# Intelligent-Driving-Laboratory/GOPS

Hardware: AMD Instinct MI355X
Metric: env-model steps/sec (batch x H), FHADP compute_gradient + update (higher is better)
Workload: dtype f32; 1 GPU; target_veh3dof_fhadp_b4096_h30; env_id=pyth_veh3dofconti, algorithm=FHADP, batch_per_gpu=4096, horizon=30, activation=elu, parallelism=dp1

## Files before the change

### gops_amd/csrc/aux_kernels.hip

```cpp
#include <algorithm>
#include "common.h"
#include "env_models.h"
#include "launchers.h"

__device__ __forceinline__ void pack_element(const float* __restrict__ W, int N, int K, int Kp,
                                             float* __restrict__ wp, float* __restrict__ wpt, int e) {
    if (e >= N * Kp) return;
    const int i = e & 3, lane = (e >> 2) & 63, blk = e >> 8;
    {
        const int kch = Kp >> 4, nt = blk / kch, c = blk - nt * kch;
        const int n = 16 * nt + (lane & 15), k = 16 * c + 4 * (lane >> 4) + i;
        wp[e] = (k < K) ? W[(size_t)n * K + k] : 0.f;
    }
    {
        const int kch = N >> 4, nt = blk / kch, c = blk - nt * kch;
        const int kin = 16 * nt + (lane & 15), nout = 16 * c + 4 * (lane >> 4) + i;
        wpt[e] = (kin < K) ? W[(size_t)nout * K + kin] : 0.f;
    }
}

__device__ __forceinline__ void pack_element_h(const float* __restrict__ W, int N, int K, int Kp16, int Kp32, int layer,
                                               _Float16* __restrict__ wph, _Float16* __restrict__ wpth, int e) {
    const int i8 = e & 7, lane = (e >> 3) & 63, blk = e >> 9, r = lane & 15, kg = lane >> 4;
    if (e < N * Kp32) {
// ... 417 lines not shown
        const f32x4 zero4 = {0.f, 0.f, 0.f, 0.f};
        if constexpr (BF3) {
            bf16x8 b[R][3];
#pragma unroll
            for (int j = 0; j < R; ++j) {
                split_frag(xra[j][0], LAST_HALF_EMPTY ? zero4 : xra[j][1], b[j]);
                load_x(next_blk, j);
            }
#pragma unroll
            for (int i = 0; i < R; ++i) {
                const f32x4 d0 = dra[i][0], d1 = LAST_HALF_EMPTY ? zero4 : dra[i][1];
                bf16x8 a[3];
                split_frag(d0, d1, a);
                bsum[i] += ((d0[0] + d0[1]) + (d0[2] + d0[3])) + ((d1[0] + d1[1]) + (d1[2] + d1[3]));
                load_d(next_blk, i);
                constexpr int PA[6] = {2, 0, 1, 1, 0, 0}, PB[6] = {0, 2, 1, 0, 1, 0};
#pragma unroll
                for (int q = 0; q < 6; ++q)
#pragma unroll
                    for (int j = 0; j < R; ++j)
                        acc[i][j] = __builtin_amdgcn_mfma_f32_16x16x32_bf16(a[PA[q]], b[j][PB[q]], acc[i][j], 0, 0, 0);
            }
        } else {
            f32x4 xc[R][2];
#pragma unroll
            for (int j = 0; j < R; ++j) {
                xc[j][0] = xra[j][0]; xc[j][1] = LAST_HALF_EMPTY ? zero4 : xra[j][1];
                load_x(next_blk, j);
            }
#pragma unroll
            for (int i = 0; i < R; ++i) {
                const f32x4 d0 = dra[i][0], d1 = LAST_HALF_EMPTY ? zero4 : dra[i][1];
                bsum[i] += ((d0[0] + d0[1]) + (d0[2] + d0[3])) + ((d1[0] + d1[1]) + (d1[2] + d1[3]));
                load_d(next_blk, i);
#pragma unroll
                for (int u = 0; u < 8; ++u)
#pragma unroll
                    for (int j = 0; j < R; ++j)
                        acc[i][j] = __builtin_amdgcn_mfma_f32_16x16x4f32(u < 4 ? d0[u & 3] : d1[u & 3], xc[j][u >> 2][u & 3], acc[i][j], 0, 0, 0);
            }
        }
    };

#pragma unroll
    for (int j = 0; j < R; ++j) load_x(blk_of(0), j);
#pragma unroll
    for (int i = 0; i < R; ++i) load_d(blk_of(0), i);
    const int nfull = odd_tail ? nblk - 1 : nblk;
    for (int c = 0; c < nfull; ++c) block.template operator()<false>(blk_of(c + 1));
    if (odd_tail) block.template operator()<true>(blk_of(nblk));
    float* pbase = part + (size_t)split * N * Kp;
#pragma unroll
    for (int i = 0; i < R; ++i)
#pragma unroll
        for (int j = 0; j < R; ++j) {
            const int k = kb + 16 * j + f;
#pragma unroll
            for (int r = 0; r < 4; ++r) {
                const int n = nb + 16 * i + 4 * g + r;
                if (n < N && k < Kp) pbase[(size_t)n * Kp + k] = acc[i][j][r];
            }
        }
    if (want_bias) {
#pragma unroll
        for (int i = 0; i < R; ++i) {
            float t = bsum[i];
            t += __shfl_xor(t, 16);
            t += __shfl_xor(t, 32);
            if (g == 0 && nb + 16 * i + f < N) part_b[(size_t)split * N + nb + 16 * i + f] = t;
        }
    }
}

#define DW_H2_SA 1.0f
#define DW_H2_LO 1.0f
__device__ __forceinline__ void split2h(const f32x4& lo4, const f32x4& hi4, float s, f16x8& ph, f16x8& pl) {
    const float s2 = s * DW_H2_LO;
    u32x4 uh, ul;
#pragma unroll
    for (int e = 0; e < 4; ++e) {
        const float x0 = e < 2 ? lo4[2 * e] : hi4[2 * e - 4], x1 = e < 2 ? lo4[2 * e + 1] : hi4[2 * e - 3];
        const f16x2 h = __builtin_bit_cast(f16x2, __builtin_amdgcn_cvt_pkrtz(x0 * s, x1 * s));
        const float r0 = fmaf((float)h[0], -DW_H2_LO, x0 * s2), r1 = fmaf((float)h[1], -DW_H2_LO, x1 * s2);
        uh[e] = __builtin_bit_cast(unsigned, h);
        ul[e] = __builtin_bit_cast(unsigned, __builtin_amdgcn_cvt_pkrtz(r0, r1));
    }
    ph = __builtin_bit_cast(f16x8, uh);
    pl = __builtin_bit_cast(f16x8, ul);
}

__device__ __forceinline__ void split2h_mix(const f32x4& lo4, const f32x4& hi4, float s, f16x8& ph, f16x8& pl) {
    u32x4 uh, ul;
#pragma unroll
    for (int e = 0; e < 4; ++e) {
        const float x0 = e < 2 ? lo4[2 * e] : hi4[2 * e - 4], x1 = e < 2 ? lo4[2 * e + 1] : hi4[2 * e - 3];
        unsigned h, l;
        asm("v_fma_mixlo_f16 %0, %1, %2, 0" : "=v"(h) : "v"(s), "v"(x0));
        asm("v_fma_mixhi_f16 %0, %1, %2, 0" : "+v"(h) : "v"(s), "v"(x1));
        asm("v_fma_mixlo_f16 %0, %1, %2, -%3 op_sel_hi:[0,0,1]" : "=v"(l) : "v"(s), "v"(x0), "v"(h));
        asm("v_fma_mixhi_f16 %0, %1, %2, -%3 op_sel:[0,0,1] op_sel_hi:[0,0,1]" : "+v"(l) : "v"(s), "v"(x1), "v"(h));
        uh[e] = h;
        ul[e] = l;
    }
    ph = __builtin_bit_cast(f16x8, uh);
    pl = __builtin_bit_cast(f16x8, ul);
}
__device__ __forceinline__ void absmax2(float& m, float a, float b) { asm("v_max3_f32 %0, |%1|, |%2|, %0" : "+v"(m) : "v"(a), "v"(b)); }

__device__ __forceinline__ float dw_delta_yardstick(const float* dscale) {
    const float dy = gptr(dscale)[1], gv = gptr(dscale)[0];
    return dy > 0.f ? dy : gv;
}

#define DWR_STAGES 2
#define DWR_STAGE_FLOATS (4 * 2048)

template <bool H2>
__global__ __launch_bounds__(NTHREADS, 2) void dw_gemm_ring_kernel(const float* __restrict__ D, int N,
                                                                    const float* __restrict__ X, int Kp,
                                                                    long long Q, int splits, int chunks_per_split,
                                                                    float* __restrict__ part,
                                                                    float* __restrict__ part_b, const float* __restrict__ dscale, int redo_guard) {
    extern __shared__ __attribute__((aligned(16))) float ring[];
    constexpr int T = 128, R = 4;
    const int tid = threadIdx.x, lane = tid & 63, wave = tid >> 6;
    const int tiles_k = (Kp + T - 1) / T, tiles = tiles_k * (N / T);
    const int xcd = blockIdx.x & 7, local = blockIdx.x >> 3;
    const int tile = local % tiles, split = (local / tiles) * 8 + xcd;
    if (split >= splits) return;
    const int tile_n = tile / tiles_k, tile_k = tile - tile_n * tiles_k;
    const int wn = wave >> 1, wk = wave & 1;
    const int f = lane & 15, g = lane >> 4;
    const bool want_bias = part_b != nullptr && tile_k == 0 && wk == 0;
    const long long nblk_all = (Q + 1) >> 1;
    const int nblk = (int)((nblk_all - split + splits - 1) / splits);
    const bool odd_tail = (Q & 1) && ((nblk_all - 1) % splits == split);

    const float* csrc = (wave < 2) ? D + (size_t)tile_n * T * 16 : X + (size_t)tile_k * T * 16;
    const size_t ctile = (size_t)((wave < 2) ? N : Kp) * 16;
    const int kvalid = (wave < 2) ? T : min(T, Kp - tile_k * T);
    auto copy_block = [&](int c, int stage) {
        const long long bq = min(((long long)split + (long long)min(c, nblk - 1) * splits) * 2 + (wave & 1), Q - 1);
        const float* src = csrc + (size_t)bq * ctile + 4 * lane;
        const float* dst = ring + stage * DWR_STAGE_FLOATS + wave * 2048;
#pragma unroll
        for (int u = 0; u < 8; ++u) {
            const int feat = u * 16 + (lane >> 2);
            async_copy16_to_lds<true>(feat < kvalid ? src + u * 256 : src + u * 256 - (size_t)(feat - (feat % kvalid)) * 16, dst + u * 256);
        }
    };

    f32x4 acc[R][R] = {};
    float bsum[R] = {0.f, 0.f, 0.f, 0.f};
    float sd = 1.f;
    if constexpr (H2) sd = f16_grad_scale(dw_delta_yardstick(dscale)) * 16.f;
    auto block = [&]<bool LAST_HALF_EMPTY, bool M2>(int stage) {
        const float* st = ring + stage * DWR_STAGE_FLOATS;
        const float* da = st + (wn * 64 + f) * 16 + 4 * g;
        const float* xa = st + 4096 + (wk * 64 + f) * 16 + 4 * g;
        const f32x4 zero4 = {0.f, 0.f, 0.f, 0.f};
        if constexpr (M2) {
            f16x8 bh[R], bl[R];
#pragma unroll
            for (int j = 0; j < R; ++j) {
                bh[j] = *reinterpret_cast<const f16x8*>(xa + 256 * j);
                bl[j] = *reinterpret_cast<const f16x8*>(xa + 256 * j + 2048);
            }
#pragma unroll
            for (int i = 0; i < R; ++i) {
                const f16x8 ah = *reinterpret_cast<const f16x8*>(da + 256 * i), al = *reinterpret_cast<const f16x8*>(da + 256 * i + 2048);
#pragma unroll
                for (int j = 0; j < R; ++j) acc[i][j] = __builtin_amdgcn_mfma_f32_16x16x32_f16(al, bh[j], acc[i][j], 0, 0, 0);
#pragma unroll
                for (int j = 0; j < R; ++j) acc[i][j] = __builtin_amdgcn_mfma_f32_16x16x32_f16(ah, bl[j], acc[i][j], 0, 0, 0);
#pragma unroll
                for (int j = 0; j < R; ++j) acc[i][j] = __builtin_amdgcn_mfma_f32_16x16x32_f16(ah, bh[j], acc[i][j], 0, 0, 0);
            }
            return;
        }
        bf16x8 b[R][3];
#pragma unroll
        for (int j = 0; j < R; ++j) {
            const f32x4 x0 = *reinterpret_cast<const f32x4*>(xa + 256 * j);
            const f32x4 x1 = LAST_HALF_EMPTY ? zero4 : *reinterpret_cast<const f32x4*>(xa + 256 * j + 2048);
            split_frag(x0, x1, b[j]);
        }
#pragma unroll
        for (int i = 0; i < R; ++i) {
            const f32x4 d0 = *reinterpret_cast<const f32x4*>(da + 256 * i);
            const f32x4 d1 = LAST_HALF_EMPTY ? zero4 : *reinterpret_cast<const f32x4*>(da + 256 * i + 2048);
            bf16x8 a[3];
            split_frag(d0, d1, a);
            bsum[i] += ((d0[0] + d0[1]) + (d0[2] + d0[3])) + ((d1[0] + d1[1]) + (d1[2] + d1[3]));
            constexpr int PA[6] = {2, 0, 1, 1, 0, 0}, PB[6] = {0, 2, 1, 0, 1, 0};
#pragma unroll
            for (int q = 0; q < 6; ++q)
#pragma unroll
                for (int j = 0; j < R; ++j)
                    acc[i][j] = __builtin_amdgcn_mfma_f32_16x16x32_bf16(a[PA[q]], b[j][PB[q]], acc[i][j], 0, 0, 0);
        }
    };

    float vmax = 0.f;
    float csum[2] = {0.f, 0.f};
    auto convert_stage = [&]<bool LAST_HALF_EMPTY>(int stage) {
        float* st = ring + stage * DWR_STAGE_FLOATS;
#pragma unroll
        for (int k = 0; k < 4; ++k) {
            const int id = tid + NTHREADS * k, op = id >> 9, fe = (id >> 2) & 127, gg = id & 3;
            float* at = st + op * 4096 + fe * 16 + 4 * gg;
            const f32x4 v0 = *reinterpret_cast<const f32x4*>(at);
            const f32x4 zero4 = {0.f, 0.f, 0.f, 0.f};
            const f32x4 v1 = LAST_HALF_EMPTY ? zero4 : *reinterpret_cast<const f32x4*>(at + 2048);
            if (k < 2) csum[k] += ((v0[0] + v0[1]) + (v0[2] + v0[3])) + ((v1[0] + v1[1]) + (v1[2] + v1[3]));
            const float sc = k < 2 ? sd : DW_H2_SA;
            const float m0 = fmaxf(fmaxf(fabsf(v0[0]), fabsf(v0[1])), fmaxf(fabsf(v0[2]), fabsf(v0[3])));
            const float m1 = fmaxf(fmaxf(fabsf(v1[0]), fabsf(v1[1])), fmaxf(fabsf(v1[2]), fabsf(v1[3])));
            vmax = fmaxf(vmax, fmaxf(m0, m1) * sc);
            f16x8 ph, pl;
            split2h(v0, v1, sc, ph, pl);
            *reinterpret_cast<f16x8*>(at) = ph;
            *reinterpret_cast<f16x8*>(at + 2048) = pl;
        }
    };
    const int nfull = odd_tail ? nblk - 1 : nblk;
    auto run = [&]<bool M2>() {
#pragma unroll
        for (int d = 0; d < DWR_STAGES - 1; ++d) copy_block(d, d);
        for (int c = 0; c < nblk; ++c) {
            asm volatile("s_waitcnt vmcnt(%0)" ::"n"(8 * (DWR_STAGES - 2)) : "memory");
            __syncthreads();
            copy_block(c + DWR_STAGES - 1, (c + DWR_STAGES - 1) % DWR_STAGES);
            if constexpr (M2) {
                if (c < nfull) convert_stage.template operator()<false>(c % DWR_STAGES);
                else convert_stage.template operator()<true>(c % DWR_STAGES);
                __syncthreads();
            }
            if (c < nfull) block.template operator()<false, M2>(c % DWR_STAGES);
            else block.template operator()<true, M2>(c % DWR_STAGES);
        }
        asm volatile("s_waitcnt vmcnt(0)" ::: "memory");
    };
    bool redone = false;
    if constexpr (H2) {
        if (tid == 0) ring[DWR_STAGES * DWR_STAGE_FLOATS] = 0.f;
        run.template operator()<true>();
        unsigned* sat = reinterpret_cast<unsigned*>(ring + DWR_STAGES * DWR_STAGE_FLOATS);
        if (!(vmax < 65504.f)) *sat = 1u;
        __syncthreads();
        if (*sat != 0u && redo_guard) {
            redone = true;
#pragma unroll
            for (int i = 0; i < R; ++i)
#pragma unroll
                for (int j = 0; j < R; ++j) acc[i][j] = f32x4{0.f, 0.f, 0.f, 0.f};
            run.template operator()<false>();
        }
    } else {
        run.template operator()<false>();
    }

    const int nb = tile_n * T + wn * 64, kb = tile_k * T + wk * 64;
    float* pbase = part + (size_t)split * N * Kp;
    const float unscale = (H2 && !redone) ? 1.f / (sd * DW_H2_SA) : 1.f;
#pragma unroll
    for (int i = 0; i < R; ++i)
#pragma unroll
        for (int j = 0; j < R; ++j) {
            const int k = kb + 16 * j + f;
            if (k >= Kp) continue;
#pragma unroll
            for (int r = 0; r < 4; ++r) {
                float v = acc[i][j][r];
                if constexpr (H2) v *= unscale;
                pbase[(size_t)(nb + 16 * i + 4 * g + r) * Kp + k] = v;
            }
        }
    if constexpr (H2) {
        if (part_b != nullptr && tile_k == 0) {
#pragma unroll
            for (int k = 0; k < 2; ++k) {
                float t = csum[k];
                t += __shfl_xor(t, 1);
                t += __shfl_xor(t, 2);
                if ((tid & 3) == 0) part_b[(size_t)split * N + tile_n * T + 64 * k + (tid >> 2)] = t;
            }
        }
    } else
    if (want_bias) {
#pragma unroll
        for (int i = 0; i < R; ++i) {
            float t = bsum[i];
            t += __shfl_xor(t, 16);
            t += __shfl_xor(t, 32);
            if (g == 0) part_b[(size_t)split * N + nb + 16 * i + f] = t;
        }
    }
}

struct DwSpec {
    static constexpr int NW = 8, NT = 512, TN = 256, T = 128;
    static constexpr int DT = TN * 16;
    static constexpr int STAGES = 3;
    static constexpr int STAGE_FLOATS = 2 * DT + 4096;
    static constexpr int PIECES = STAGE_FLOATS / 256 / NW;
    static constexpr size_t lds_bytes() { return (size_t)STAGES * STAGE_FLOATS * sizeof(float) + 16; }
};

struct DwSpecGeo {
    const float* dbase;
    const float* xbase;
    float* pbase;
    long long Q;
    int N, Kp, split, splits, nblk, nfull, xgroups, tile_n, tile_k;
};
__device__ __forceinline__ void dw_spec_copy(const DwSpecGeo& G, float* ring, int c, int stage, int wave, int lane) {
    constexpr int T = DwSpec::T, TN = DwSpec::TN, PC = DwSpec::PIECES;
    const long long b0 = ((long long)G.split + (long long)c * G.splits) * 2;
    float* dst = ring + stage * DwSpec::STAGE_FLOATS + wave * PC * 256;
#pragma unroll
    for (int u = 0; u < PC; ++u) {
        const int pc = wave * PC + u;
        const bool isx = pc >= 2 * (TN / 16);
        const int q = isx ? pc - 2 * (TN / 16) : pc, per = isx ? T / 16 : TN / 16;
        const int st_tile = q / per;
        int grp = q - st_tile * per;
        if (isx && grp >= G.xgroups) grp %= G.xgroups;
        const size_t bq = (size_t)min(b0 + st_tile, G.Q - 1);
        const float* src = (isx ? G.xbase + bq * ((size_t)G.Kp * 16) : G.dbase + bq * ((size_t)G.N * 16)) + grp * 256 + 4 * lane;
        async_copy16_to_lds<true>(src, dst + u * 256);
    }
}
__device__ __forceinline__ void dw_spec_store(const DwSpecGeo& G, const f32x4 (&acc)[8][4], int wn, int wk, int f, int g, float unscale) {
    const int nb = G.tile_n * DwSpec::TN + wn * 128, kb = G.tile_k * DwSpec::T + wk * 64;
#pragma unroll
    for (int i = 0; i < 8; ++i)
#pragma unroll
        for (int j = 0; j < 4; ++j) {
            const int k = kb + 16 * j + f;
            if (k >= G.Kp) continue;
#pragma unroll
            for (int r = 0; r < 4; ++r) G.pbase[(size_t)(nb + 16 * i + 4 * g + r) * G.Kp + k] = acc[i][j][r] * unscale;
        }
}
__device__ __attribute__((noinline)) void dw_spec_exact_pass(const DwSpecGeo G, float* ring) {
    constexpr int DT = DwSpec::DT, SF = DwSpec::STAGE_FLOATS, NST = DwSpec::STAGES;
    const int tid = threadIdx.x, lane = tid & 63, wave = tid >> 6;
    const bool mul_wave = wave >= 4;
    const int mw = wave & 3, wn = mw >> 1, wk = mw & 1, f = lane & 15, g = lane >> 4;
    f32x4 acc[8][4] = {};
    dw_spec_copy(G, ring, 0, 0, wave, lane);
    if (G.nblk > 1) dw_spec_copy(G, ring, 1, 1, wave, lane);
    for (int c = 0; c < G.nblk; ++c) {
        asm volatile("s_waitcnt vmcnt(0)" ::: "memory");
        __syncthreads();
        if (c + 2 < G.nblk) dw_spec_copy(G, ring, c + 2, (c + 2) % NST, wave, lane);
        if (mul_wave) {
            const bool half_empty = c >= G.nfull;
            const float* st = ring + (c % NST) * SF;
            const float* da = st + (wn * 128 + f) * 16 + 4 * g;
            const float* xa = st + 2 * DT + (wk * 64 + f) * 16 + 4 * g;
            const f32x4 zero4 = {0.f, 0.f, 0.f, 0.f};
            bf16x8 b[4][3];
#pragma unroll
            for (int j = 0; j < 4; ++j) {
                const f32x4 x0 = *reinterpret_cast<const f32x4*>(xa + 256 * j);
                const f32x4 x1 = half_empty ? zero4 : *reinterpret_cast<const f32x4*>(xa + 256 * j + 2048);
                split_frag(x0, x1, b[j]);
            }
#pragma unroll
            for (int i = 0; i < 8; ++i) {
                const f32x4 d0 = *reinterpret_cast<const f32x4*>(da + 256 * i);
                const f32x4 d1 = half_empty ? zero4 : *reinterpret_cast<const f32x4*>(da + 256 * i + DT);
                bf16x8 a[3];
                split_frag(d0, d1, a);
                constexpr int PA[6] = {2, 0, 1, 1, 0, 0}, PB[6] = {0, 2, 1, 0, 1, 0};
#pragma unroll
                for (int q = 0; q < 6; ++q)
#pragma unroll
                    for (int j = 0; j < 4; ++j)
                        acc[i][j] = __builtin_amdgcn_mfma_f32_16x16x32_bf16(a[PA[q]], b[j][PB[q]], acc[i][j], 0, 0, 0);
                __builtin_amdgcn_sched_barrier(0);
            }
        }
    }
    if (mul_wave) dw_spec_store(G, acc, wn, wk, f, g, 1.f);
}

__global__ __launch_bounds__(512, 1) void dw_gemm_spec_kernel(const float* __restrict__ D, int N, const float* __restrict__ X, int Kp, long long Q,
                                                              int splits, float* __restrict__ part, float* __restrict__ part_b,
                                                              const float* __restrict__ dscale, int guard) {
    extern __shared__ __attribute__((aligned(16))) float ring[];
    constexpr int T = DwSpec::T, TN = DwSpec::TN, DT = DwSpec::DT, SF = DwSpec::STAGE_FLOATS, NST = DwSpec::STAGES;
    const int tid = threadIdx.x, lane = tid & 63, wave = tid >> 6;
    const bool mul_wave = wave >= 4;
    const int tiles_k = (Kp + T - 1) / T, tiles = tiles_k * (N / TN);
    const int xcd = blockIdx.x & 7, local = blockIdx.x >> 3;
    const int tile = local % tiles, split = (local / tiles) * 8 + xcd;
    if (split >= splits) return;
    const int f = lane & 15, g = lane >> 4;
    DwSpecGeo G;
    G.tile_n = tile / tiles_k;
    G.tile_k = tile - G.tile_n * tiles_k;
    G.N = N; G.Kp = Kp; G.Q = Q; G.split = split; G.splits = splits;
    const long long nblk_all = (Q + 1) >> 1;
    G.nblk = (int)((nblk_all - split + splits - 1) / splits);
    const bool odd_tail = (Q & 1) && ((nblk_all - 1) % splits == split);
    G.nfull = odd_tail ? G.nblk - 1 : G.nblk;
    G.xgroups = min(T, Kp - G.tile_k * T) >> 4;
    G.dbase = D + (size_t)G.tile_n * TN * 16;
    G.xbase = X + (size_t)G.tile_k * T * 16;
    G.pbase = part + (size_t)split * N * Kp;
    const int nblk = G.nblk, nfull = G.nfull;

    const int mw = wave & 3, wn = mw >> 1, wk = mw & 1;
    const float sd = f16_grad_scale(dw_delta_yardstick(dscale)) * 16.f;
    float vmax = 0.f, vmax_d = 0.f, vmax_x = 0.f;
    float csum[4] = {0.f, 0.f, 0.f, 0.f};
    const bool want_csum = part_b != nullptr && G.tile_k == 0;

    unsigned* sat = reinterpret_cast<unsigned*>(ring + NST * SF);
    if (tid == 0) *sat = 0u;
    struct Raw { f32x4 v[6][2]; };
    Raw r0, r1;
    const int gg = tid & 3;
    long long lofs[6];
#pragma unroll
    for (int k = 0; k < 6; ++k) {
        const bool isd = k < 4;
        int fe = (tid >> 2) + 64 * (isd ? k : k - 4);
        if (!isd) { int grp = fe >> 4; if (grp >= G.xgroups) grp %= G.xgroups; fe = (grp << 4) | (fe & 15); }
        lofs[k] = (long long)fe * 16 + 4 * gg;
    }
    const size_t dtile = (size_t)N * 16, xtile = (size_t)Kp * 16;
    auto load_block = [&](int c, Raw& r) {
        const size_t q0 = (size_t)(((long long)split + (long long)c * splits) * 2);
        const bool second = c < nfull;
        const f32x4 zero4 = {0.f, 0.f, 0.f, 0.f};
#pragma unroll
        for (int k = 0; k < 6; ++k) {
            const float* base = (k < 4 ? G.dbase + q0 * dtile : G.xbase + q0 * xtile) + lofs[k];
            r.v[k][0] = DW_STREAM_LOAD(reinterpret_cast<const f32x4*>(base));
            r.v[k][1] = second ? DW_STREAM_LOAD(reinterpret_cast<const f32x4*>(base + (k < 4 ? dtile : xtile))) : zero4;
        }
    };
    auto convert_block = [&](const Raw& r, int stage) {
        float* st = ring + stage * SF;
#pragma unroll
        for (int k = 0; k < 6; ++k) {
            const bool isd = k < 4;
            const int fe = (tid >> 2) + 64 * (isd ? k : k - 4), second = isd ? DT : 2048;
            float* at = st + (isd ? 0 : 2 * DT) + fe * 16 + 4 * gg;
            const f32x4 v0 = r.v[k][0], v1 = r.v[k][1];
            if (isd && want_csum) csum[k & 3] += ((v0[0] + v0[1]) + (v0[2] + v0[3])) + ((v1[0] + v1[1]) + (v1[2] + v1[3]));
            float& vm = isd ? vmax_d : vmax_x;
            absmax2(vm, v0[0], v0[1]); absmax2(vm, v0[2], v0[3]);
            absmax2(vm, v1[0], v1[1]); absmax2(vm, v1[2], v1[3]);
            f16x8 ph, pl;
            split2h_mix(v0, v1, isd ? sd : DW_H2_SA, ph, pl);
            *reinterpret_cast<f16x8*>(at) = ph;
            *reinterpret_cast<f16x8*>(at + second) = pl;
        }
    };
    if (mul_wave) {
        f32x4 acc[8][4] = {};
        auto block_h2 = [&](int stage) {
            const float* st = ring + stage * SF;
            const float* da = st + (wn * 128 + f) * 16 + 4 * g;
            const float* xa = st + 2 * DT + (wk * 64 + f) * 16 + 4 * g;
            f16x8 bh[4], bl[4];
    #pragma unroll
            for (int j = 0; j < 4; ++j) {
                bh[j] = *reinterpret_cast<const f16x8*>(xa + 256 * j);
                bl[j] = *reinterpret_cast<const f16x8*>(xa + 256 * j + 2048);
            }
            f16x8 ah = *reinterpret_cast<const f16x8*>(da), al = *reinterpret_cast<const f16x8*>(da + DT);
    #pragma unroll
            for (int i = 0; i < 8; ++i) {
                f16x8 nh = ah, nl = al;
                if (i + 1 < 8) {
                    nh = *reinterpret_cast<const f16x8*>(da + 256 * (i + 1));
                    nl = *reinterpret_cast<const f16x8*>(da + 256 * (i + 1) + DT);
                }
                __builtin_amdgcn_sched_barrier(0);
    #pragma unroll
                for (int j = 0; j < 4; ++j) acc[i][j] = __builtin_amdgcn_mfma_f32_16x16x32_f16(al, bh[j], acc[i][j], 0, 0, 0);
    #pragma unroll
                for (int j = 0; j < 4; ++j) acc[i][j] = __builtin_amdgcn_mfma_f32_16x16x32_f16(ah, bl[j], acc[i][j], 0, 0, 0);
    #pragma unroll
                for (int j = 0; j < 4; ++j) acc[i][j] = __builtin_amdgcn_mfma_f32_16x16x32_f16(ah, bh[j], acc[i][j], 0, 0, 0);
                __builtin_amdgcn_sched_barrier(0);
                ah = nh; al = nl;
            }
        };

        __syncthreads();
        for (int c = 0; c < nblk; ++c) {
            block_h2(c % NST);
            __syncthreads();
        }
        __syncthreads();
        if (*sat != 0u && guard) {
            dw_spec_exact_pass(G, ring);
            return;
        }
        dw_spec_store(G, acc, wn, wk, f, g, 1.f / (sd * DW_H2_SA));
        return;
    }
    load_block(0, r0);
    if (nblk > 1) load_block(1, r1);
    convert_block(r0, 0);
    if (nblk > 2) load_block(2, r0);
    if (nblk > 1) convert_block(r1, 1);
    if (nblk > 3) load_block(3, r1);
    __syncthreads();
    auto iteration = [&](int c, Raw& r) {
        if (c + 2 < nblk) {
            convert_block(r, (c + 2) % NST);
            if (c + 4 < nblk) load_block(c + 4, r);
        }
        __syncthreads();
    };
    for (int c = 0; c < nblk; c += 2) {
        iteration(c, r0);
        if (c + 1 < nblk) iteration(c + 1, r1);
    }
    if (!mul_wave) {
        vmax = fmaxf(vmax_d * sd, vmax_x * DW_H2_SA);
        if (!(vmax < 65504.f)) *sat = 1u;
        if (want_csum) {
#pragma unroll
            for (int k = 0; k < 4; ++k) {
                float t = csum[k];
                t += __shfl_xor(t, 1);
                t += __shfl_xor(t, 2);
                if ((tid & 3) == 0) part_b[(size_t)split * N + G.tile_n * TN + 64 * k + (tid >> 2)] = t;
            }
        }
    }
    __syncthreads();
    if (*sat != 0u && guard) {
        dw_spec_exact_pass(G, ring);
        return;
    }
}

#define DWK_U 2
__global__ __launch_bounds__(NTHREADS, 3) void dw_skinny_kernel(const float* __restrict__ D, int N, const float* __restrict__ X, long long Q,
                                                                 int splits, float* __restrict__ part, float* __restrict__ part_b) {
    const int tid = threadIdx.x, lane = tid & 63, wave = tid >> 6;
    const int f = lane & 15, g = lane >> 4;
    const int ngroups = (N + 255) / 256;
    const int xcd = blockIdx.x & 7, local = blockIdx.x >> 3;
    const int grp = local % ngroups, split = (local / ngroups) * 8 + xcd;
    if (split >= splits) return;
    int doff[4], nfeat[4];
#pragma unroll
    for (int i = 0; i < 4; ++i) {
        nfeat[i] = 256 * grp + 16 * (wave + 4 * i);
        doff[i] = min(nfeat[i] + f, N - 1) * 16 + 4 * g;
    }
    const int xoff = f * 16 + 4 * g;
    const GLOBAL_AS float* Dg = gptr(D);
    const GLOBAL_AS float* Xg = gptr(X);
    const size_t dtile = (size_t)N * 16;
    struct Batch { f32x4 d[DWK_U][4]; f32x4 x[DWK_U]; };
    auto load = [&](long long q0, Batch& b) {
#pragma unroll
        for (int u = 0; u < DWK_U; ++u) {
            const long long q = q0 + (long long)u * splits;
            const size_t qq = (size_t)min(q, Q - 1);
#pragma unroll
            for (int i = 0; i < 4; ++i) b.d[u][i] = DW_STREAM_LOAD(reinterpret_cast<const GLOBAL_AS f32x4*>(Dg + qq * dtile + doff[i]));
            b.x[u] = DW_STREAM_LOAD(reinterpret_cast<const GLOBAL_AS f32x4*>(Xg + qq * 256 + xoff));
        }
    };
    f32x4 acc[4] = {};
    float bsum[4] = {0.f, 0.f, 0.f, 0.f};
    auto mul = [&](long long q0, const Batch& b) {
#pragma unroll
        for (int u = 0; u < DWK_U; ++u) {
            const bool live = q0 + (long long)u * splits < Q;
            f32x4 x = b.x[u];
#pragma unroll
            for (int e = 0; e < 4; ++e) x[e] = live ? x[e] : 0.f;
#pragma unroll
            for (int i = 0; i < 4; ++i) {
                const f32x4 d = b.d[u][i];
                bsum[i] += live ? (d[0] + d[1]) + (d[2] + d[3]) : 0.f;
#pragma unroll
                for (int e = 0; e < 4; ++e) acc[i] = __builtin_amdgcn_mfma_f32_16x16x4f32(d[e], x[e], acc[i], 0, 0, 0);
            }
        }
    };
    const long long stride = (long long)DWK_U * splits;
    Batch b0, b1;
    load(split, b0);
    for (long long q = split; q < Q; q += 2 * stride) {
        load(q + stride, b1);
        mul(q, b0);
        load(q + 2 * stride, b0);
        mul(q + stride, b1);
    }
    float* pbase = part + (size_t)split * N * 16;
#pragma unroll
    for (int i = 0; i < 4; ++i) {
        if (nfeat[i] >= N) continue;
#pragma unroll
        for (int r = 0; r < 4; ++r) pbase[(size_t)(nfeat[i] + 4 * g + r) * 16 + f] = acc[i][r];
        if (part_b != nullptr) {
            float t = bsum[i];
            t += __shfl_xor(t, 16);
            t += __shfl_xor(t, 32);
            if (g == 0) part_b[(size_t)split * N + nfeat[i] + f] = t;
        }
    }
}

#define DWH_T 128
#define DWH_PLANE (8 * DWH_T * 8)

typedef unsigned u32x2 __attribute__((ext_vector_type(2)));

__global__ __launch_bounds__(NTHREADS, 2) void dw_gemm_f16_kernel(const _Float16* __restrict__ D, int N,
                                                                   const _Float16* __restrict__ X, int Kp,
                                                                   long long S, int splits, int chunks_per_split,
                                                                   float* __restrict__ part,
                                                                   float* __restrict__ part_b) {
    __shared__ __attribute__((aligned(16))) _Float16 As[DWH_PLANE];
    __shared__ __attribute__((aligned(16))) _Float16 Bs[DWH_PLANE];
    const int tid = threadIdx.x, lane = tid & 63, wave = tid >> 6;
    const int tiles_k = (Kp + DWH_T - 1) / DWH_T, tiles = tiles_k * ((N + DWH_T - 1) / DWH_T);
    const int xcd = blockIdx.x & 7, local = blockIdx.x >> 3;
    const int tile = local % tiles, split = (local / tiles) * 8 + xcd;
    if (split >= splits) return;
    const int tile_n = tile / tiles_k, tile_k = tile - tile_n * tiles_k;
    const int n0 = tile_n * DWH_T, k0 = tile_k * DWH_T;
    const long long s_begin = (long long)split * chunks_per_split * DWH_SC;
    const int wn = wave >> 1, wk = wave & 1;

    const int c8 = ((lane >> 1) & 7) | (((lane >> 4) & 1) << 3);
    const int s4 = (lane & 1) | (((lane >> 5) & 1) << 1) | (wave << 2);
    int wofs[8];
#pragma unroll
    for (int i = 0; i < 8; ++i) {
        const int n = 8 * c8 + i, nsw = n ^ ((n >> 3) & 7);
        wofs[i] = (((s4 >> 1) * DWH_T + nsw) << 3) + ((s4 & 1) << 2);
    }
    const bool want_bias = part_b != nullptr && tile_k == 0;

    f32x4 acc[4][4] = {};
    u32x4 dreg[4], xreg[4];
    float bsum[8] = {0.f, 0.f, 0.f, 0.f, 0.f, 0.f, 0.f, 0.f};

    auto gload = [&](long long s0) {
#pragma unroll
        for (int r = 0; r < 4; ++r) {
            const long long srow = s0 + 4 * s4 + r;
            const int n = n0 + 8 * c8, k = k0 + 8 * c8;
            const u32x4 z = {0u, 0u, 0u, 0u};
            dreg[r] = (srow < S && n < N) ? *reinterpret_cast<const u32x4*>(D + srow * N + n) : z;
            xreg[r] = (srow < S && k < Kp) ? *reinterpret_cast<const u32x4*>(X + srow * Kp + k) : z;
        }
    };
    auto lstore = [&]<bool SUM>(const u32x4& q0, const u32x4& q1, const u32x4& q2, const u32x4& q3, _Float16* base) {
        #pragma unroll
        for (int w = 0; w < 4; ++w) {
            const unsigned r0w = q0[w], r1w = q1[w], r2w = q2[w], r3w = q3[w];
            const unsigned lo01 = (r0w & 0xffffu) | (r1w << 16), lo23 = (r2w & 0xffffu) | (r3w << 16);
            const unsigned hi01 = (r0w >> 16) | (r1w & 0xffff0000u), hi23 = (r2w >> 16) | (r3w & 0xffff0000u);
            { const u32x2 v = {lo01, lo23}; *reinterpret_cast<u32x2*>(base + wofs[2 * w]) = v; }
            { const u32x2 v = {hi01, hi23}; *reinterpret_cast<u32x2*>(base + wofs[2 * w + 1]) = v; }
            if (SUM && want_bias) {
                const f16x2 a0 = __builtin_bit_cast(f16x2, lo01), a1 = __builtin_bit_cast(f16x2, lo23);
                const f16x2 b0 = __builtin_bit_cast(f16x2, hi01), b1 = __builtin_bit_cast(f16x2, hi23);
                bsum[2 * w] += ((float)a0[0] + (float)a0[1]) + ((float)a1[0] + (float)a1[1]);
                bsum[2 * w + 1] += ((float)b0[0] + (float)b0[1]) + ((float)b1[0] + (float)b1[1]);
            }
        }
    };
    auto frag = [&](const _Float16* base, int ks, int col) {
        const int nsw = col ^ ((col >> 3) & 7);
        return *reinterpret_cast<const f16x8*>(base + (((4 * ks + (lane >> 4)) * DWH_T + nsw) << 3));
    };

    gload(s_begin);
    for (int c = 0; c < chunks_per_split; ++c) {
        __syncthreads();
        lstore.template operator()<true>(dreg[0], dreg[1], dreg[2], dreg[3], As);
        lstore.template operator()<false>(xreg[0], xreg[1], xreg[2], xreg[3], Bs);
        __syncthreads();
        if (c + 1 < chunks_per_split) gload(s_begin + (long long)(c + 1) * DWH_SC);
#pragma unroll
        for (int ks = 0; ks < 2; ++ks) {
            f16x8 b[4];
#pragma unroll
            for (int j = 0; j < 4; ++j) b[j] = frag(Bs, ks, wk * 64 + 16 * j + (lane & 15));
#pragma unroll
            for (int i = 0; i < 4; ++i) {
                const f16x8 a = frag(As, ks, wn * 64 + 16 * i + (lane & 15));
#pragma unroll
                for (int j = 0; j < 4; ++j) acc[i][j] = __builtin_amdgcn_mfma_f32_16x16x32_f16(a, b[j], acc[i][j], 0, 0, 0);
            }
        }
    }
    float* pbase = part + (size_t)split * N * Kp;
#pragma unroll
    for (int i = 0; i < 4; ++i)
#pragma unroll
        for (int j = 0; j < 4; ++j) {
            const int k = k0 + wk * 64 + 16 * j + (lane & 15);
#pragma unroll
            for (int r = 0; r < 4; ++r) {
                const int n = n0 + wn * 64 + 16 * i + 4 * (lane >> 4) + r;
                if (n < N && k < Kp) pbase[(size_t)n * Kp + k] = acc[i][j][r];
            }
        }
    if (want_bias) {
        __syncthreads();
        float* red = reinterpret_cast<float*>(As);
#pragma unroll
        for (int i = 0; i < 8; ++i) red[s4 * DWH_T + 8 * c8 + i] = bsum[i];
        __syncthreads();
        if (tid < DWH_T && n0 + tid < N) {
            float t = 0.f;
#pragma unroll
            for (int q = 0; q < 16; ++q) t += red[q * DWH_T + tid];
            part_b[(size_t)split * N + n0 + tid] = t;
        }
    }
}

__global__ __launch_bounds__(NTHREADS) void dw_out_h_kernel(const float* __restrict__ dy, const _Float16* __restrict__ h, int K, int A,
                                                            long long S, long long per_split, float* __restrict__ part,
                                                            float* __restrict__ part_b) {
    __shared__ __attribute__((aligned(16))) float red[4][GOPS_MAX_ACT][256];
    __shared__ float redb[4][GOPS_MAX_ACT];
    const int split = blockIdx.x, tid = threadIdx.x, c8 = tid & 31, sl = tid >> 5, wave = tid >> 6;
    const long long s0 = split * per_split, s1 = min(S, s0 + per_split);
    const int nblk = K >> 3;
    for (int cb0 = 0; cb0 < nblk; cb0 += 32) {
        const int cb = cb0 + c8;
        const bool col_ok = cb < nblk;
        float acc[GOPS_MAX_ACT][8] = {};
        float accb[GOPS_MAX_ACT] = {0.f, 0.f, 0.f, 0.f};
        if (col_ok) {
            const GLOBAL_AS _Float16* hp = gptr(h) + 8 * cb;
#pragma unroll 4
            for (long long sidx = s0 + sl; sidx < s1; sidx += 8) {
                const f32x4 g = *gptr(reinterpret_cast<const f32x4*>(dy) + sidx);
                const f16x8 hv = *reinterpret_cast<const GLOBAL_AS f16x8*>(hp + sidx * K);
#pragma unroll
                for (int a = 0; a < GOPS_MAX_ACT; ++a) {
#pragma unroll
                    for (int e = 0; e < 8; ++e) acc[a][e] = fmaf(g[a], (float)hv[e], acc[a][e]);
                    accb[a] += g[a];
                }
            }
        }
#pragma unroll
        for (int a = 0; a < GOPS_MAX_ACT; ++a) {
#pragma unroll
            for (int e = 0; e < 8; ++e) acc[a][e] += __shfl_xor(acc[a][e], 32);
            accb[a] += __shfl_xor(accb[a], 32);
        }
        if ((tid & 32) == 0) {
#pragma unroll
            for (int a = 0; a < GOPS_MAX_ACT; ++a) {
                *reinterpret_cast<f32x4*>(&red[wave][a][8 * c8]) = f32x4{acc[a][0], acc[a][1], acc[a][2], acc[a][3]};
                *reinterpret_cast<f32x4*>(&red[wave][a][8 * c8 + 4]) = f32x4{acc[a][4], acc[a][5], acc[a][6], acc[a][7]};
            }
            if (c8 == 0 && cb0 == 0)
                for (int a = 0; a < GOPS_MAX_ACT; ++a) redb[wave][a] = accb[a];
        }
        __syncthreads();
        const int k = 8 * cb0 + tid;
        if (k < K)
            for (int a = 0; a < A; ++a)
                part[((size_t)split * A + a) * K + k] = (red[0][a][tid] + red[1][a][tid]) + (red[2][a][tid] + red[3][a][tid]);
        if (tid == 0 && cb0 == 0)
            for (int a = 0; a < A; ++a) part_b[(size_t)split * A + a] = (redb[0][a] + redb[1][a]) + (redb[2][a] + redb[3][a]);
        __syncthreads();
    }
}

__global__ __launch_bounds__(NTHREADS) void dw_out_fm_kernel(const float* __restrict__ dy, const float* __restrict__ h, int K, int A,
                                                             long long Q, long long tiles_per_split,
                                                             float* __restrict__ part, float* __restrict__ part_b) {
    const int split = blockIdx.x;
    const long long q0 = split * tiles_per_split, q1 = min(Q, q0 + tiles_per_split);
    for (int k = threadIdx.x; k < ((K + NTHREADS - 1) / NTHREADS) * NTHREADS; k += NTHREADS) {
        const bool col_ok = k < K;
        const int kc = col_ok ? k : K - 1;
        float acc[GOPS_MAX_ACT] = {0.f, 0.f, 0.f, 0.f}, accb[GOPS_MAX_ACT] = {0.f, 0.f, 0.f, 0.f};
        for (long long qb = q0; qb < q1; qb += 2) {
            f32x4 hv[2][4];
#pragma unroll
            for (int u = 0; u < 2; ++u) {
                const long long q = min(qb + u, q1 - 1);
#pragma unroll
                for (int rg = 0; rg < 4; ++rg) hv[u][rg] = ld4(gptr(h) + ((size_t)q * K + kc) * 16 + 4 * rg);
            }
#pragma unroll
            for (int u = 0; u < 2; ++u) {
                if (qb + u < q1) {
                    const f32x4* gp = reinterpret_cast<const f32x4*>(dy) + (size_t)(qb + u) * 16;
#pragma unroll
                    for (int m = 0; m < 16; ++m) {
                        const f32x4 g = gp[m];
#pragma unroll
                        for (int a = 0; a < GOPS_MAX_ACT; ++a) { acc[a] += g[a] * hv[u][m >> 2][m & 3]; accb[a] += g[a]; }
                    }
                }
            }
        }
        if (col_ok) {
            for (int a = 0; a < A; ++a) part[((size_t)split * A + a) * K + k] = acc[a];
            if (k == 0)
                for (int a = 0; a < A; ++a) part_b[(size_t)split * A + a] = accb[a];
        }
    }
}

static_assert(DW_SC == 2 * TB, "a K-block of the fp32 dW GEMMs is two sample tiles (nblk_all = (Q + 1) >> 1)");
static inline int cdiv(int a, int b) { return (a + b - 1) / b; }

bool dw_skinny_ok(int N, int Kp) { return Kp == 16 && (N % 16) == 0; }

DwLayer plan_dw(int N, int K, int Kp, long long S, bool f16, int wg_target) {
    DwLayer L;
    L.N = N, L.K = K, L.Kp = Kp, L.S = S, L.ld = Kp;
    L.tile = (f16 || (N >= 128 && Kp >= 128)) ? 128 : 64;
    const int counted = (!f16 && dw_skinny_ok(N, Kp)) ? cdiv(N, 256) : cdiv(N, L.tile) * cdiv(Kp, L.tile);
    const int sc = f16 ? DWH_SC : DW_SC;
    const long long chunks = (S + sc - 1) / sc;
    if (wg_target < 1) wg_target = 512;
    long long splits = (wg_target + counted - 1) / counted;
    if (splits > chunks) splits = chunks;
    if (splits < 1) splits = 1;
    L.chunks_per_split = (int)((chunks + splits - 1) / splits);
    L.splits = (int)((chunks + L.chunks_per_split - 1) / L.chunks_per_split);
    L.slab_w = (size_t)L.splits * N * Kp;
// ... 674 lines not shown
```

Before: 202.9 million env-model steps/s.

## Split dW staging work between producer and MFMA waves in specialized kernel

In the warp-specialized dW kernel, the producer waves used to load and convert all six chunks per block (four delta chunks and two activation chunks) into the f16 hi/lo LDS ring, while the MFMA waves only computed. Now the producer waves handle the delta chunks and the MFMA waves load and convert the activation chunks themselves, interleaved with their MFMA work. The saturation check and bias column-sum logic is split the same way. The goal is to shorten the producer's critical path so the MFMA waves stall less at barriers. The cost is extra register pressure and global-load latency on the MFMA waves, which already hold a large accumulator array.

```diff
diff --git a/gops_amd/csrc/aux_kernels.hip b/gops_amd/csrc/aux_kernels.hip
--- a/gops_amd/csrc/aux_kernels.hip
+++ b/gops_amd/csrc/aux_kernels.hip
@@ -743,6 +743,7 @@
     static constexpr int NW = 8, NT = 512, TN = 256, T = 128;
     static constexpr int DT = TN * 16;
     static constexpr int STAGES = 3;
+    static constexpr int KSPLIT = 4;
     static constexpr int STAGE_FLOATS = 2 * DT + 4096;
     static constexpr int PIECES = STAGE_FLOATS / 256 / NW;
     static constexpr size_t lds_bytes() { return (size_t)STAGES * STAGE_FLOATS * sizeof(float) + 16; }
@@ -856,41 +857,40 @@
 
     const int mw = wave & 3, wn = mw >> 1, wk = mw & 1;
     const float sd = f16_grad_scale(dw_delta_yardstick(dscale)) * 16.f;
-    float vmax = 0.f, vmax_d = 0.f, vmax_x = 0.f;
+    float vmax_d = 0.f, vmax_x = 0.f;
     float csum[4] = {0.f, 0.f, 0.f, 0.f};
     const bool want_csum = part_b != nullptr && G.tile_k == 0;
 
     unsigned* sat = reinterpret_cast<unsigned*>(ring + NST * SF);
     if (tid == 0) *sat = 0u;
     struct Raw { f32x4 v[6][2]; };
-    Raw r0, r1;
-    const int gg = tid & 3;
+    const int ct = tid & 255, gg = ct & 3;
     long long lofs[6];
 #pragma unroll
     for (int k = 0; k < 6; ++k) {
         const bool isd = k < 4;
-        int fe = (tid >> 2) + 64 * (isd ? k : k - 4);
+        int fe = (ct >> 2) + 64 * (isd ? k : k - 4);
         if (!isd) { int grp = fe >> 4; if (grp >= G.xgroups) grp %= G.xgroups; fe = (grp << 4) | (fe & 15); }
         lofs[k] = (long long)fe * 16 + 4 * gg;
     }
     const size_t dtile = (size_t)N * 16, xtile = (size_t)Kp * 16;
-    auto load_block = [&](int c, Raw& r) {
+    auto load_block = [&]<int K0, int K1>(int c, Raw& r) {
         const size_t q0 = (size_t)(((long long)split + (long long)c * splits) * 2);
         const bool second = c < nfull;
         const f32x4 zero4 = {0.f, 0.f, 0.f, 0.f};
 #pragma unroll
-        for (int k = 0; k < 6; ++k) {
+        for (int k = K0; k < K1; ++k) {
             const float* base = (k < 4 ? G.dbase + q0 * dtile : G.xbase + q0 * xtile) + lofs[k];
             r.v[k][0] = DW_STREAM_LOAD(reinterpret_cast<const f32x4*>(base));
             r.v[k][1] = second ? DW_STREAM_LOAD(reinterpret_cast<const f32x4*>(base + (k < 4 ? dtile : xtile))) : zero4;
         }
     };
-    auto convert_block = [&](const Raw& r, int stage) {
+    auto convert_block = [&]<int K0, int K1>(const Raw& r, int stage) {
         float* st = ring + stage * SF;
 #pragma unroll
-        for (int k = 0; k < 6; ++k) {
+        for (int k = K0; k < K1; ++k) {
             const bool isd = k < 4;
-            const int fe = (tid >> 2) + 64 * (isd ? k : k - 4), second = isd ? DT : 2048;
+            const int fe = (ct >> 2) + 64 * (isd ? k : k - 4), second = isd ? DT : 2048;
             float* at = st + (isd ? 0 : 2 * DT) + fe * 16 + 4 * gg;
             const f32x4 v0 = r.v[k][0], v1 = r.v[k][1];
             if (isd && want_csum) csum[k & 3] += ((v0[0] + v0[1]) + (v0[2] + v0[3])) + ((v1[0] + v1[1]) + (v1[2] + v1[3]));
@@ -903,6 +903,34 @@
             *reinterpret_cast<f16x8*>(at + second) = pl;
         }
     };
+    auto first_blocks = [&]<int K0, int K1>(Raw& a, Raw& b) {
+        load_block.template operator()<K0, K1>(0, a);
+        if (nblk > 1) load_block.template operator()<K0, K1>(1, b);
+        convert_block.template operator()<K0, K1>(a, 0);
+        if (nblk > 2) load_block.template operator()<K0, K1>(2, a);
+        if (nblk > 1) convert_block.template operator()<K0, K1>(b, 1);
+        if (nblk > 3) load_block.template operator()<K0, K1>(3, b);
+    };
+    auto next_block = [&]<int K0, int K1>(int c, Raw& r) {
+        if (c + 2 < nblk) {
+            convert_block.template operator()<K0, K1>(r, (c + 2) % NST);
+            if (c + 4 < nblk) load_block.template operator()<K0, K1>(c + 4, r);
+        }
+    };
+    auto verdict = [&]<int K0, int K1>() {
+        const float vmax = fmaxf(vmax_d * sd, vmax_x * DW_H2_SA);
+        if (!(vmax < 65504.f)) *sat = 1u;
+        if (want_csum) {
+#pragma unroll
+            for (int k = K0; k < (K1 < 4 ? K1 : 4); ++k) {
+                float t = csum[k];
+                t += __shfl_xor(t, 1);
+                t += __shfl_xor(t, 2);
+                if (gg == 0) part_b[(size_t)split * N + G.tile_n * TN + 64 * k + (ct >> 2)] = t;
+            }
+        }
+    };
+    constexpr int KS = DwSpec::KSPLIT;
     if (mul_wave) {
         f32x4 acc[8][4] = {};
         auto block_h2 = [&](int stage) {
@@ -935,11 +963,19 @@
             }
         };
 
+        Raw x0, x1;
+        first_blocks.template operator()<KS, 6>(x0, x1);
         __syncthreads();
-        for (int c = 0; c < nblk; ++c) {
+        auto iteration = [&](int c, Raw& r) {
             block_h2(c % NST);
+            next_block.template operator()<KS, 6>(c, r);
             __syncthreads();
-        }
+        };
+        for (int c = 0; c < nblk; c += 2) {
+            iteration(c, x0);
+            if (c + 1 < nblk) iteration(c + 1, x1);
+        }
+        verdict.template operator()<KS, 6>();
         __syncthreads();
         if (*sat != 0u && guard) {
             dw_spec_exact_pass(G, ring);
@@ -948,37 +984,18 @@
         dw_spec_store(G, acc, wn, wk, f, g, 1.f / (sd * DW_H2_SA));
         return;
     }
-    load_block(0, r0);
-    if (nblk > 1) load_block(1, r1);
-    convert_block(r0, 0);
-    if (nblk > 2) load_block(2, r0);
-    if (nblk > 1) convert_block(r1, 1);
-    if (nblk > 3) load_block(3, r1);
+    Raw r0, r1;
+    first_blocks.template operator()<0, KS>(r0, r1);
     __syncthreads();
     auto iteration = [&](int c, Raw& r) {
-        if (c + 2 < nblk) {
-            convert_block(r, (c + 2) % NST);
-            if (c + 4 < nblk) load_block(c + 4, r);
-        }
+        next_block.template operator()<0, KS>(c, r);
         __syncthreads();
     };
     for (int c = 0; c < nblk; c += 2) {
         iteration(c, r0);
         if (c + 1 < nblk) iteration(c + 1, r1);
     }
-    if (!mul_wave) {
-        vmax = fmaxf(vmax_d * sd, vmax_x * DW_H2_SA);
-        if (!(vmax < 65504.f)) *sat = 1u;
-        if (want_csum) {
-#pragma unroll
-            for (int k = 0; k < 4; ++k) {
-                float t = csum[k];
-                t += __shfl_xor(t, 1);
-                t += __shfl_xor(t, 2);
-                if ((tid & 3) == 0) part_b[(size_t)split * N + G.tile_n * TN + 64 * k + (tid >> 2)] = t;
-            }
-        }
-    }
+    verdict.template operator()<0, KS>();
     __syncthreads();
     if (*sat != 0u && guard) {
         dw_spec_exact_pass(G, ring);
```

After: 201.6 million env-model steps/s. No clear change (-0.7%).
